# DakeQQ/Voice-Activity-Detection-VAD-ONNX

Hardware: NVIDIA B200
Metric: RTFx (audio-hours/sec) (higher is better)
Workload: dtype f32

## Files before the change

### voice-activity-detection-vad-onnx_b200/csrc/stft_tc.cu

```cuda
#include "tc_ptx.cuh"

namespace vadx {

constexpr int kStNPad = 80;
constexpr int kStTerms = 2;
constexpr int kStLead = 8;
constexpr int kStJ = 2;
constexpr int kStSlices = 2 * kStJ;
constexpr int kStStages = 3;
constexpr int kStLoaderWarps = 16;
constexpr int kStOutLd = 44;

struct StftTcArgs {
  const int16_t* X;
  int64_t in_stride;
  int64_t L;
  int64_t S;
  int n_frames, hop;
  int h16;
  int n_q;
  int tq;
  int rows;
  int slice_units;
  int n_st;
  const uint8_t* Wimg;
  float* P;
  int64_t ldp;
  int n_bins, kc, n_k16, n_tiles, vec_p;
  int pad_left;
  const float* mean;
  const int* mean_int;
  const float* dc;
  int n_edge_lo, t_edge_hi;
  float power_scale;
  int stage_out;
  unsigned backoff_ld, backoff_epi;
  int debug;
};

__device__ __forceinline__ uint32_t bf16x2_lo(uint32_t w) {
  const float a = __uint_as_float(0x4B000000u | (w & 0xffu)) - 8388608.0f;
  const float b = __uint_as_float(0x4B000000u | ((w >> 16) & 0xffu)) - 8388608.0f;
  return __byte_perm(__float_as_uint(a), __float_as_uint(b), 0x7632);
}
__device__ __forceinline__ uint32_t bf16x2_hi(uint32_t w) {
  const uint32_t ha = (((w >> 8) & 0xffu) ^ 0x80u);
  const uint32_t hb = (((w >> 24) & 0xffu) ^ 0x80u);
  const float a = fmaf(__uint_as_float(0x4B000000u | ha), 256.0f, -(8388608.0f + 128.0f) * 256.0f);
  const float b = fmaf(__uint_as_float(0x4B000000u | hb), 256.0f, -(8388608.0f + 128.0f) * 256.0f);
  return __byte_perm(__float_as_uint(a), __float_as_uint(b), 0x7632);
}

__device__ __forceinline__ uint32_t f16x2_lo(uint32_t w) {
  const uint32_t m = (w & 0x00ff00ffu) | 0x64006400u;
  uint32_t r;
  asm("sub.rn.f16x2 %0, %1, %2;" : "=r"(r) : "r"(m), "r"(0x64006400u));
  return r;
}
__device__ __forceinline__ uint32_t f16x2_hi(uint32_t w) {
  const uint32_t m = (((w >> 8) & 0x00ff00ffu) ^ 0x00800080u) | 0x64006400u;
  uint32_t r;
  asm("sub.rn.f16x2 %0, %1, %2;" : "=r"(r) : "r"(m), "r"(0x64806480u));
  asm("mul.rn.f16x2 %0, %1, %2;" : "=r"(r) : "r"(r), "r"(0x5c005c00u));
  return r;
}

__device__ __forceinline__ void split17(int d, float& hi, float& lo) {
  lo = __uint_as_float(0x4B000000u | (uint32_t)(d & 255)) - 8388608.0f;
  const uint32_t h = (uint32_t)((d >> 8) + 256);
  hi = fmaf(__uint_as_float(0x4B000000u | h), 256.0f, -(8388608.0f + 256.0f) * 256.0f);
}

template <bool EX, bool F16>
__global__ void __launch_bounds__((kStLoaderWarps + 5) * 32, 1) stft_power_tc_kernel(const StftTcArgs g) {
  constexpr int kStEpiWarp0 = kStLoaderWarps, kStMmaWarp = kStLoaderWarps + 4;
  extern __shared__ __align__(1024) uint8_t smem_raw[];
  uint8_t* w_smem = smem_raw;
  const uint32_t img_bytes = kStNPad * 128u;
  const int w_bytes = g.kc * kStTerms * (int)img_bytes;
  uint8_t* a_smem = w_smem + w_bytes;
  const uint32_t slice_bytes = (uint32_t)g.slice_units * 16u;
  const uint32_t term_bytes = kStSlices * slice_bytes;
  const uint32_t stage_bytes = 2u * term_bytes;
  uint64_t* bars = reinterpret_cast<uint64_t*>(a_smem + (size_t)kStStages * stage_bytes);
  uint32_t* tmem_slot = reinterpret_cast<uint32_t*>(bars + 13);
  float* out_stage = reinterpret_cast<float*>(bars + 16);

  const int warp = threadIdx.x >> 5, lane = threadIdx.x & 31;
  const uint32_t bar0 = smem_u32(bars);
  auto full_bar = [&](int s) { return bar0 + 8u * s; };
  auto empty_bar = [&](int s) { return bar0 + 8u * (4 + s); };
  auto tfull_bar = [&](int b) { return bar0 + 8u * (8 + b); };
  auto tempty_bar = [&](int b) { return bar0 + 8u * (10 + b); };
  const uint32_t wbar = bar0 + 8u * 12;
  constexpr int kAccN = 2 * kStNPad;
  constexpr uint32_t kTmemCols = 512;

  if (threadIdx.x == 0) {
    for (int s = 0; s < kStStages; ++s) {
      mbar_init(full_bar(s), kStLoaderWarps);
      mbar_init(empty_bar(s), 1);
    }
    for (int b = 0; b < 2; ++b) {
      mbar_init(tfull_bar(b), 1);
      mbar_init(tempty_bar(b), 4);
    }
    mbar_init(wbar, 1);
    asm volatile("fence.mbarrier_init.release.cluster;" ::: "memory");
  }
  if (warp == kStMmaWarp) {
    asm volatile("tcgen05.alloc.cta_group::1.sync.aligned.shared::cta.b32 [%0], %1;" ::"r"(smem_u32(tmem_slot)),
                 "r"(kTmemCols)
                 : "memory");
    asm volatile("tcgen05.relinquish_alloc_permit.cta_group::1.sync.aligned;" ::: "memory");
  }
  tc_fence_before();
  __syncthreads();
  tc_fence_after();
  const uint32_t tmem_base = *tmem_slot;
  const int ntile = blockIdx.y;

  if (warp == kStMmaWarp) {
    if (lane == 0) {
      mbar_expect_tx(wbar, (uint32_t)w_bytes);
      const uint8_t* src = g.Wimg + (size_t)ntile * w_bytes;
      for (int t = 0; t < g.kc * kStTerms; ++t) bulk_g2s(smem_u32(w_smem) + t * img_bytes, src + (size_t)t * img_bytes, img_bytes, wbar);
      mbar_wait(wbar, 0);
      const uint32_t idesc = F16 ? umma_idesc_f16(kAccN) : umma_idesc_bf16(kAccN);
      const uint64_t dw = umma_desc_sw128(smem_u32(w_smem));
      const uint64_t da0 = umma_desc_noswz(smem_u32(a_smem), slice_bytes, 128u);
      const uint32_t chunk_units = (kStTerms * img_bytes) >> 4, lo_units = term_bytes >> 4, stage_units = stage_bytes >> 4;
      const uint32_t col_units = (2u * slice_bytes) >> 4;
      const int h16 = g.h16, n_k16 = g.n_k16;
      const uint32_t lo_on = (g.debug & 4) ? 0u : 1u;
      constexpr bool kBurst = F16 && !EX;
      auto b_desc = [&](int k) { return dw + (uint64_t)((uint32_t)(k >> 2) * chunk_units + 2u * (uint32_t)(k & 3)); };
      int stage = 0;
      uint32_t phase = 0;
      int it = 0;
      for (int tile = blockIdx.x; tile < g.n_tiles; tile += gridDim.x, ++it) {
        const int b = it & 1;
        const uint32_t use = (uint32_t)(it >> 1);
        mbar_wait(tempty_bar(b), (use & 1u) ^ 1u);
        tc_fence_after();
        const uint32_t d_tmem = tmem_base + (uint32_t)(b * kAccN);
        for (int st = 0; st < g.n_st; ++st) {
          mbar_wait(full_bar(stage), phase);
          tc_fence_after();
          const uint64_t da_st = da0 + (uint64_t)stage * stage_units;
#pragma unroll
          for (int jj = 0; jj < kStJ; ++jj) {
            const int j = st * kStJ + jj;
            if (j >= h16) break;
            const uint64_t da_j = da_st + (uint64_t)jj * col_units;
            if (kBurst) {
              for (int q0 = 0, k = j; k < n_k16; q0 += 3, k += 3 * h16) {
                const int n_pairs = 1 + (k + h16 < n_k16 ? 1 : 0) + (k + 2 * h16 < n_k16 ? 1 : 0);
                umma_split_x3(d_tmem, da_j + (uint64_t)q0, 1u, lo_units, b_desc(k), b_desc(k + h16), b_desc(k + 2 * h16),
                              idesc, k ? 1u : 0u, n_pairs, lo_on);
              }
            } else {
              for (int q = 0, k = j; k < n_k16; ++q, k += h16) {
                const uint64_t da = da_j + (uint64_t)q;
                if (g.debug & 4) umma_bf16(d_tmem, da, b_desc(k), idesc, k ? 1u : 0u);
                else umma_x2(d_tmem, da, da + lo_units, b_desc(k), idesc, k ? 1u : 0u);
              }
            }
          }
          umma_commit(empty_bar(stage));
          if (++stage == kStStages) { stage = 0; phase ^= 1u; }
        }
        umma_commit(tfull_bar(b));
      }
    }
  } else if (warp < kStLoaderWarps) {
    constexpr int kRowsPerPass = kStLoaderWarps * 32 / kStSlices;
    constexpr int kPasses = 2;
    const int t = threadIdx.x;
    const int sl = t % kStSlices;
    const int r_in = t / kStSlices;
    const int16_t* xs_n[kPasses];
    int h0_n[kPasses];
    uint32_t rok_n = 0u;
    int tile_cached = -1;
    struct Seq { int tile, st; };
    auto valid = [&](const Seq& q) { return q.tile < g.n_tiles; };
    auto advance = [&](Seq& q) { if (++q.st == g.n_st) { q.st = 0; q.tile += gridDim.x; } };
    const int n_groups = 2 * g.h16;
    auto issue = [&](const Seq& q, uint4* raw, uint32_t& msk) {
      msk = 0u;
      if (q.tile != tile_cached) {
        rok_n = 0u;
#pragma unroll
        for (int pass = 0; pass < kPasses; ++pass) {
          const int r = pass * kRowsPerPass + r_in;
          const int64_t slot = (int64_t)q.tile * kTcBM + r;
          const int64_t s = slot / g.tq;
          const int h = (int)(slot - s * g.tq);
          const bool ok = r < g.rows && s < g.S;
          xs_n[pass] = g.X + (ok ? s : 0) * g.in_stride;
          h0_n[pass] = h * g.hop - (EX ? g.pad_left : 0) - kStLead;
          if (ok) rok_n |= 1u << pass;
        }
        tile_cached = q.tile;
      }
      const int grp = q.st * kStSlices + sl;
#pragma unroll
      for (int pass = 0; pass < kPasses; ++pass) {
        const int i0 = h0_n[pass] + 8 * grp;
        uint4 v = make_uint4(0u, 0u, 0u, 0u);
        if (((rok_n >> pass) & 1u) && grp < n_groups && i0 >= 0 && i0 + 7 < g.L) {
          v = __ldg(reinterpret_cast<const uint4*>(xs_n[pass] + i0));
          msk |= 1u << pass;
        }
        raw[pass] = v;
      }
    };
    int stage = 0;
    uint32_t phase = 0;
    int mi_c[kPasses];
#pragma unroll
    for (int pass = 0; pass < kPasses; ++pass) mi_c[pass] = 0;
    int tile_cached_c = -1;
    auto consume = [&](const Seq& q, const uint4* raw, uint32_t msk) {
      if (EX && g.mean_int && q.tile != tile_cached_c) {
#pragma unroll
        for (int pass = 0; pass < kPasses; ++pass) {
          const int64_t s = ((int64_t)q.tile * kTcBM + pass * kRowsPerPass + r_in) / g.tq;
          mi_c[pass] = s < g.S ? __ldg(g.mean_int + s) : 0;
        }
        tile_cached_c = q.tile;
      }
      mbar_wait(empty_bar(stage), phase ^ 1u, g.backoff_ld);
      uint8_t* st_hi = a_smem + (size_t)stage * stage_bytes + sl * slice_bytes;
      uint8_t* st_lo = st_hi + term_bytes;
      if (!(g.debug & 8) && q.st * kStSlices + sl < n_groups)
#pragma unroll
      for (int pass = 0; pass < kPasses; ++pass) {
        const int r = pass * kRowsPerPass + r_in;
        if (r >= g.rows) break;
        const uint32_t wds[4] = {raw[pass].x, raw[pass].y, raw[pass].z, raw[pass].w};
        uint32_t hi[4], lo[4];
        if (EX && g.mean_int) {
          const int mi = ((msk >> pass) & 1u) ? mi_c[pass] : 0;
#pragma unroll
          for (int j = 0; j < 4; ++j) {
            const uint32_t w = wds[j];
            const int a = ((int)(w << 16) >> 16) - mi;
            const int b = ((int)w >> 16) - mi;
            float ah, al, bh, bl;
            split17(a, ah, al);
            split17(b, bh, bl);
            hi[j] = __byte_perm(__float_as_uint(ah), __float_as_uint(bh), 0x7632);
            lo[j] = __byte_perm(__float_as_uint(al), __float_as_uint(bl), 0x7632);
          }
        } else {
#pragma unroll
        for (int j = 0; j < 4; ++j) {
          const uint32_t w = wds[j];
          hi[j] = F16 ? f16x2_hi(w) : bf16x2_hi(w);
          lo[j] = F16 ? f16x2_lo(w) : bf16x2_lo(w);
        }
        }
        *reinterpret_cast<uint4*>(st_hi + r * 16) = make_uint4(hi[0], hi[1], hi[2], hi[3]);
        *reinterpret_cast<uint4*>(st_lo + r * 16) = make_uint4(lo[0], lo[1], lo[2], lo[3]);
      }
      if (!(g.debug & 16)) fence_proxy_async();
      __syncwarp();
      if (lane == 0) mbar_arrive(full_bar(stage));
      if (++stage == kStStages) { stage = 0; phase ^= 1u; }
    };
    constexpr int kStBufs = EX ? 4 : 6;
    uint4 bufs[kStBufs][kPasses];
    uint32_t msks[kStBufs];
#pragma unroll
    for (int i = 0; i < kStBufs; ++i) msks[i] = 0u;
    Seq nxt{(int)blockIdx.x, 0}, cur{(int)blockIdx.x, 0};
#pragma unroll
    for (int i = 0; i < kStBufs - 1; ++i)
      if (valid(nxt)) { issue(nxt, bufs[i], msks[i]); advance(nxt); }
    while (valid(cur)) {
#pragma unroll
      for (int i = 0; i < kStBufs; ++i) {
        constexpr int kPrev = kStBufs - 1;
        if (valid(nxt)) { issue(nxt, bufs[(i + kPrev) % kStBufs], msks[(i + kPrev) % kStBufs]); advance(nxt); }
        consume(cur, bufs[i], msks[i]); advance(cur);
        if (!valid(cur)) break;
      }
    }
  } else {
    const int q = warp - kStEpiWarp0;
    int it = 0;
    const int f0 = ntile * (kStNPad / 2);
    for (int tile = blockIdx.x; tile < g.n_tiles; tile += gridDim.x, ++it) {
      const int b = it & 1;
      const uint32_t use = (uint32_t)(it >> 1);
      mbar_wait(tfull_bar(b), use & 1u, g.backoff_epi);
      tc_fence_after();
      const int64_t slot = (int64_t)tile * kTcBM + q * 32 + lane;
      const int64_t sidx = slot / g.tq;
      const int t = (int)(slot - sidx * g.tq);
      const bool row_ok = sidx < g.S && t < g.n_frames;
      const int64_t row = row_ok ? sidx * g.n_frames + t : -1;
      const uint32_t taddr = tmem_base + ((uint32_t)(q * 32) << 16) + (uint32_t)(b * kAccN);
      float* const my_out = out_stage + (size_t)q * 32 * kStOutLd;
      float m_row = 0.f, x_last = 0.f;
      const float* dc_row = nullptr;
      const float* tail_row = nullptr;
      if (EX && g.dc && row_ok) {
        const int n_edge = g.n_edge_lo + (g.n_frames - g.t_edge_hi);
        if (g.mean) {
          m_row = __ldg(g.mean + sidx);
          const int e = t < g.n_edge_lo ? 1 + t : (t >= g.t_edge_hi ? 1 + g.n_edge_lo + (t - g.t_edge_hi) : 0);
          dc_row = g.dc + ((size_t)e * gridDim.y + ntile) * kStNPad;
        }
        if (t >= g.t_edge_hi) {
          x_last = (float)((int)__ldg(g.X + sidx * g.in_stride + (g.L - 1)) - (g.mean_int ? __ldg(g.mean_int + sidx) : 0));
          tail_row = g.dc + ((size_t)(1 + n_edge + (t - g.t_edge_hi)) * gridDim.y + ntile) * kStNPad;
        }
      }
#pragma unroll
      for (int c0 = 0; c0 < kStNPad; c0 += 16) {
        float v[16], v2[16];
        tmem_ld16(taddr + (uint32_t)c0, v);
        tmem_ld16(taddr + (uint32_t)(kStNPad + c0), v2);
#pragma unroll
        for (int j = 0; j < 16; ++j) v[j] += v2[j];
        if (!row_ok || (g.debug & 1)) continue;
        if (EX && dc_row) {
#pragma unroll
          for (int j = 0; j < 16; ++j) v[j] = fmaf(-m_row, __ldg(dc_row + c0 + j), v[j]);
        }
        if (EX && tail_row) {
#pragma unroll
          for (int j = 0; j < 16; ++j) v[j] = fmaf(x_last, __ldg(tail_row + c0 + j), v[j]);
        }
        float* out = g.P + row * g.ldp + f0 + c0 / 2;
        float pw[8];
#pragma unroll
        for (int j = 0; j < 8; ++j) pw[j] = (v[2 * j] * v[2 * j] + v[2 * j + 1] * v[2 * j + 1]) * g.power_scale;
        const int fb = f0 + c0 / 2;
        if (g.stage_out) {
          float4* d4 = reinterpret_cast<float4*>(my_out + lane * kStOutLd + c0 / 2);
          d4[0] = make_float4(pw[0], pw[1], pw[2], pw[3]);
          d4[1] = make_float4(pw[4], pw[5], pw[6], pw[7]);
        } else if (g.vec_p && fb + 7 < g.n_bins) {
          reinterpret_cast<float4*>(out)[0] = make_float4(pw[0], pw[1], pw[2], pw[3]);
          reinterpret_cast<float4*>(out)[1] = make_float4(pw[4], pw[5], pw[6], pw[7]);
        } else {
#pragma unroll
          for (int j = 0; j < 8; ++j)
            if (fb + j < g.n_bins) out[j] = pw[j];
        }
      }
      tc_fence_before();
      __syncwarp();
      if (lane == 0) mbar_arrive(tempty_bar(b));
      if (g.stage_out && !(g.debug & 1)) {
        constexpr int kC4 = kStNPad / 8;
#pragma unroll
        for (int itr = 0; itr < kC4; ++itr) {
          const int idx = itr * 32 + lane;
          const int r = idx / kC4, c4 = idx - r * kC4;
          const long long grow = __shfl_sync(0xffffffffu, (long long)row, r);
          const int fbin = f0 + c4 * 4;
          if (grow >= 0 && fbin < g.n_bins) {
            const float4 val = *reinterpret_cast<const float4*>(my_out + r * kStOutLd + c4 * 4);
            float* out = g.P + grow * g.ldp + fbin;
            if (fbin + 3 < g.n_bins) {
              *reinterpret_cast<float4*>(out) = val;
            } else {
              out[0] = val.x;
              if (fbin + 1 < g.n_bins) out[1] = val.y;
              if (fbin + 2 < g.n_bins) out[2] = val.z;
            }
          }
        }
        __syncwarp();
      }
    }
  }
  tc_fence_before();
  __syncthreads();
  if (warp == kStMmaWarp) {
    tc_fence_after();
    asm volatile("tcgen05.dealloc.cta_group::1.sync.aligned.b32 %0, %1;" ::"r"(tmem_base), "r"(kTmemCols) : "memory");
  }
}

struct StftTcRing {
  int n_q, rows, slice_units;
  size_t bytes;
};
static StftTcRing stft_tc_ring(int n_k16, int h16) {
  StftTcRing r{};
  r.n_q = (n_k16 - 1) / h16 + 1;
  r.rows = kTcBM + r.n_q - 1;
  r.slice_units = r.rows + ((2 - r.rows % 4) + 4) % 4;
  r.bytes = (size_t)kStStages * 2 * kStSlices * r.slice_units * 16;
  return r;
}

struct StftTcShape {
  int kc, n_k16, n_ntiles;
  size_t tile_bytes, img_bytes, smem_bytes, stage_bytes;
  bool ok;
};
StftTcShape stft_tc_shape(int n_taps, int n_bins, int hop = 16) {
  StftTcShape s{};
  const int k_used = n_taps + kStLead;
  s.kc = (int)ceil_div(k_used, kTcBK);
  s.n_k16 = (int)ceil_div(k_used, 16);
  s.n_ntiles = (int)ceil_div(2 * n_bins, kStNPad);
  s.tile_bytes = (size_t)s.kc * kStTerms * kStNPad * 128;
  s.img_bytes = s.tile_bytes * s.n_ntiles;
  s.smem_bytes = s.tile_bytes + stft_tc_ring(s.n_k16, std::max(1, hop / 16)).bytes + 16 * 8;
  s.stage_bytes = (size_t)4 * 32 * kStOutLd * sizeof(float);
  s.ok = s.smem_bytes <= (size_t)kTcSmemBudget;
  return s;
}

}

using namespace vadx;

extern "C" int vadx_stft_tc_supported(int n_taps, int n_bins) { return stft_tc_shape(n_taps, n_bins).ok ? 1 : 0; }

extern "C" int vadx_pack_stft_basis_tc(const float* h_basis, int ld_basis, int n_taps, int n_bins, double preemph,
                                       double scale, void* h_img, size_t img_capacity, size_t* img_bytes) {
  return vadx_pack_stft_basis_tc_fmt(h_basis, ld_basis, n_taps, n_bins, preemph, scale, VADX_TC_FMT_BF16, h_img, img_capacity,
                                     img_bytes);
}

extern "C" int vadx_pack_stft_basis_tc_fmt(const float* h_basis, int ld_basis, int n_taps, int n_bins, double preemph,
                                           double scale, int operand_format, void* h_img, size_t img_capacity,
                                           size_t* img_bytes) {
  VADX_REQUIRE(h_basis && img_bytes && n_taps > 0 && n_bins > 0 && ld_basis >= 2 * n_bins,
               "vadx_pack_stft_basis_tc: bad argument");
  VADX_REQUIRE(operand_format == VADX_TC_FMT_BF16 || operand_format == VADX_TC_FMT_F16, "vadx_pack_stft_basis_tc: operand format %d",
               operand_format);
  const bool f16 = operand_format == VADX_TC_FMT_F16;
  StftTcShape s = stft_tc_shape(n_taps, n_bins);
  VADX_REQUIRE(s.ok, "vadx_pack_stft_basis_tc: %d taps x %d bins does not fit the tensor-core DFT", n_taps, n_bins);
  *img_bytes = s.img_bytes;
  if (!h_img) return VADX_OK;
  VADX_REQUIRE(img_capacity >= s.img_bytes, "vadx_pack_stft_basis_tc: image buffer too small");
  uint8_t* img = static_cast<uint8_t*>(h_img);
  memset(img, 0, s.img_bytes);
  const int n_cols = 2 * n_bins;
  const size_t term = (size_t)kStNPad * 128;
  for (int col = 0; col < n_cols; ++col) {
    const int nt = col / kStNPad, r = col % kStNPad;
    for (int k = 0; k < n_taps + kStLead; ++k) {
      const int n0 = k - kStLead, n1 = k - kStLead + 1;
      double v = 0.0;
      if (n0 >= 0 && n0 < n_taps) v += (double)h_basis[(size_t)n0 * ld_basis + col];
      if (n1 >= 0 && n1 < n_taps) v -= preemph * (double)h_basis[(size_t)n1 * ld_basis + col];
      v *= scale;
      const float f = (float)v;
      const uint16_t b0 = f16 ? f16_rn_host(f) : bf16_rn_host(f);
      const float r1 = (float)(v - (double)(f16 ? f16_to_f_host(b0) : bf16_to_f_host(b0)));
      const uint16_t b1 = f16 ? f16_rn_host(r1) : bf16_rn_host(r1);
      const int c = k / kTcBK, kk = k % kTcBK;
      uint8_t* base = img + (size_t)nt * s.tile_bytes + (size_t)(c * kStTerms) * term + sw128_offset(r, kk);
      memcpy(base, &b0, 2);
      memcpy(base + term, &b1, 2);
    }
  }
  return VADX_OK;
}

extern "C" int vadx_pack_stft_dc_tc(const float* h_basis, int ld_basis, int n_taps, int n_bins, double preemph, double scale,
                                    int64_t n_samples, int hop, int pad_left, int n_frames, float* h_tables,
                                    size_t capacity_floats, size_t* n_floats, int* n_edge_lo, int* t_edge_hi) {
  VADX_REQUIRE(h_basis && n_floats && n_edge_lo && t_edge_hi && n_taps > 0 && n_bins > 0 && hop > 0 && pad_left >= 0 &&
                   n_frames > 0 && ld_basis >= 2 * n_bins,
               "vadx_pack_stft_dc_tc: bad argument");
  StftTcShape s = stft_tc_shape(n_taps, n_bins);
  VADX_REQUIRE(s.ok, "vadx_pack_stft_dc_tc: shape not supported");
  int lo = 0;
  while (lo < n_frames && (int64_t)lo * hop - pad_left < 1) ++lo;
  int hi = n_frames;
  while (hi > lo && (int64_t)(hi - 1) * hop - pad_left + n_taps - 1 >= n_samples) --hi;
  *n_edge_lo = lo;
  *t_edge_hi = hi;
  const int n_edge = lo + (n_frames - hi);
  const size_t ncp = (size_t)s.n_ntiles * kStNPad;
  *n_floats = (size_t)(1 + n_edge + (n_frames - hi)) * ncp;
  if (!h_tables) return VADX_OK;
  VADX_REQUIRE(capacity_floats >= *n_floats, "vadx_pack_stft_dc_tc: table buffer too small");
  memset(h_tables, 0, *n_floats * sizeof(float));
  auto fill = [&](float* row, int64_t origin, bool interior) {
    for (int col = 0; col < 2 * n_bins; ++col) {
      double acc = 0.0;
      for (int n = 0; n < n_taps; ++n) {
        const int64_t i = origin + n;
        double coef = interior ? 1.0 - preemph : (i < 0 || i >= n_samples ? 0.0 : (i == 0 ? 1.0 : 1.0 - preemph));
        acc += coef * (double)h_basis[(size_t)n * ld_basis + col];
      }
      row[col] = (float)(acc * scale);
    }
  };
  fill(h_tables, 0, true);
  int e = 1;
  for (int t = 0; t < lo; ++t, ++e) fill(h_tables + (size_t)e * ncp, (int64_t)t * hop - pad_left, false);
  for (int t = hi; t < n_frames; ++t, ++e) fill(h_tables + (size_t)e * ncp, (int64_t)t * hop - pad_left, false);
  for (int t = hi; t < n_frames; ++t, ++e) {
    const int64_t n_l = n_samples - ((int64_t)t * hop - pad_left);
    if (n_l < 0 || n_l >= n_taps) continue;
    float* row = h_tables + (size_t)e * ncp;
    for (int col = 0; col < 2 * n_bins; ++col) row[col] = (float)(preemph * scale * (double)h_basis[(size_t)n_l * ld_basis + col]);
  }
  return VADX_OK;
}

namespace vadx {
__global__ void __launch_bounds__(256) stream_mean_i16_kernel(const int16_t* __restrict__ x, int64_t in_stride, int64_t n,
                                                              float* __restrict__ mean_frac, int* __restrict__ mean_int) {
  const int64_t s = blockIdx.x;
  const int16_t* p = x + s * in_stride;
  long long acc = 0;
  for (int64_t i = threadIdx.x; i < n; i += blockDim.x) acc += (long long)__ldg(p + i);
  __shared__ long long part[8];
#pragma unroll
  for (int off = 16; off > 0; off >>= 1) acc += __shfl_xor_sync(0xffffffffu, acc, off);
  if ((threadIdx.x & 31) == 0) part[threadIdx.x >> 5] = acc;
  __syncthreads();
  if (threadIdx.x == 0) {
    long long t = 0;
    for (int w = 0; w < 8; ++w) t += part[w];
    const double m = (double)t / (double)n;
    const int mi = (int)llrint(m);
    mean_int[s] = mi;
    mean_frac[s] = (float)(m - (double)mi);
  }
}
}

extern "C" int vadx_stream_mean_i16(const int16_t* d_audio, int64_t in_stride, int64_t n_samples, int64_t n_streams,
                                    float* d_mean_frac, int32_t* d_mean_int, void* stream) {
  StageTimer _timer(VADX_STAGE_PREP, (cudaStream_t)stream, "stream_mean_i16_kernel", 2.0 * n_streams * n_samples);
  VADX_REQUIRE(d_audio && d_mean_frac && d_mean_int && n_samples > 0 && in_stride >= n_samples && n_streams >= 0,
               "vadx_stream_mean_i16: bad argument");
  if (n_streams == 0) return VADX_OK;
  stream_mean_i16_kernel<<<(unsigned)n_streams, 256, 0, (cudaStream_t)stream>>>(d_audio, in_stride, n_samples, d_mean_frac,
                                                                                d_mean_int);
  return after_launch("vadx_stream_mean_i16");
}

extern "C" int vadx_stft_power_tc_i16(const int16_t* d_audio, int64_t in_stride, int64_t n_samples, int64_t n_streams,
                                      int n_frames, int hop, int n_taps, const void* d_img, int n_bins, float* d_power,
                                      int64_t ld_power, void* stream) {
  VADX_REQUIRE((int64_t)(n_frames - 1) * hop + n_taps <= n_samples,
               "vadx_stft_power_tc_i16: frames must lie inside the %lld samples of a stream", (long long)n_samples);
  return vadx_stft_power_tc_i16_ex(d_audio, in_stride, n_samples, n_streams, n_frames, hop, n_taps, d_img, n_bins, d_power,
                                   ld_power, 0, nullptr, nullptr, nullptr, 0, n_frames, 1.0f, VADX_TC_FMT_BF16, stream);
}

extern "C" int vadx_stft_power_tc_i16_ex(const int16_t* d_audio, int64_t in_stride, int64_t n_samples, int64_t n_streams,
                                         int n_frames, int hop, int n_taps, const void* d_img, int n_bins, float* d_power,
                                         int64_t ld_power, int pad_left, const float* d_mean_frac, const int32_t* d_mean_int,
                                         const float* d_dc_tables, int n_edge_lo, int t_edge_hi, float power_scale,
                                         int operand_format, void* stream) {
  const float* d_mean = d_mean_frac;
  VADX_REQUIRE(operand_format == VADX_TC_FMT_BF16 || (operand_format == VADX_TC_FMT_F16 && !d_mean_frac),
               "vadx_stft_power_tc_i16: fp16 operands cannot carry the mean-removed (17-bit) samples");
  VADX_REQUIRE((d_mean_frac == nullptr) == (d_mean_int == nullptr), "vadx_stft_power_tc_i16: mean needs both its parts");
  StageTimer _timer(VADX_STAGE_STFT, (cudaStream_t)stream, "stft_power_tc_kernel",
                    2.0 * n_streams * n_samples + 4.0 * n_streams * n_frames * n_bins,
                    2.0 * n_streams * n_frames * n_taps * 2.0 * n_bins);
  VADX_REQUIRE(d_audio && d_img && d_power, "vadx_stft_power_tc_i16: null pointer");
  VADX_REQUIRE(n_streams >= 0 && n_frames > 0 && hop > 0 && n_taps > 0 && n_bins > 0 && ld_power >= n_bins,
               "vadx_stft_power_tc_i16: bad shape");
  VADX_REQUIRE(in_stride >= n_samples && pad_left >= 0 && (pad_left % 8) == 0 && (n_samples % 8) == 0,
               "vadx_stft_power_tc_i16: stride shorter than the stream, or pad_left / n_samples not a multiple of 8");
  const bool leaves_stream = pad_left > 0 || (int64_t)(n_frames - 1) * hop - pad_left + n_taps > n_samples;
  VADX_REQUIRE(!(d_mean || leaves_stream) || (d_dc_tables && n_edge_lo >= 0 && t_edge_hi >= n_edge_lo && t_edge_hi <= n_frames),
               "vadx_stft_power_tc_i16: padded frames / DC removal need the tables of vadx_pack_stft_dc_tc");
  VADX_REQUIRE((hop % 16) == 0,
               "vadx_stft_power_tc_i16: hop %d is not a multiple of 16 samples (frames are read as shifted rows of 16-sample "
               "hop slices); use vadx_stft_power_f32", hop);
  VADX_REQUIRE((in_stride % 8) == 0 && aligned16(d_audio) && aligned16(d_img),
               "vadx_stft_power_tc_i16: stream stride must be a multiple of 8 samples, pointers 16-byte aligned");
  StftTcShape s = stft_tc_shape(n_taps, n_bins, hop);
  VADX_REQUIRE(s.ok, "vadx_stft_power_tc_i16: shape not supported");
  if (n_streams == 0) return VADX_OK;
  static PerDevice per_device;
  int n_sm = 148;
  VADX_TRY(per_device.ensure(&n_sm, [] {
    cudaError_t e = cudaSuccess;
    auto opt_in = [&](auto kern) {
      if (e == cudaSuccess) e = cudaFuncSetAttribute(kern, cudaFuncAttributeMaxDynamicSharedMemorySize, kTcSmemBudget);
    };
    opt_in(stft_power_tc_kernel<false, false>);
    opt_in(stft_power_tc_kernel<true, false>);
    opt_in(stft_power_tc_kernel<false, true>);
    opt_in(stft_power_tc_kernel<true, true>);
    return e;
  }));
  const StftTcRing ring = stft_tc_ring(s.n_k16, hop / 16);
  StftTcArgs g{};
  g.X = d_audio; g.in_stride = in_stride; g.L = n_samples; g.S = n_streams; g.n_frames = n_frames; g.hop = hop;
  g.h16 = hop / 16; g.n_q = ring.n_q; g.tq = n_frames + ring.n_q - 1; g.rows = ring.rows; g.slice_units = ring.slice_units;
  g.n_st = (int)ceil_div(g.h16, kStJ);
  g.Wimg = static_cast<const uint8_t*>(d_img); g.P = d_power; g.ldp = ld_power;
  g.n_bins = n_bins; g.kc = s.kc; g.n_k16 = s.n_k16;
  g.pad_left = pad_left; g.mean = d_mean; g.mean_int = d_mean_int; g.dc = d_dc_tables; g.power_scale = power_scale; g.n_edge_lo = n_edge_lo; g.t_edge_hi = t_edge_hi;
  g.vec_p = ((ld_power & 3) == 0) && aligned16(d_power);
  {
    static const int dbg = ab_env("VADX_TC_DEBUG", 0);
    g.debug = dbg;
  }
  static const int opt = ab_env("VADX_ST_OPT", 2);
  {
    static const int bl = ab_env("VADX_TC_BACKOFF_LD", 64);
    static const int be = ab_env("VADX_TC_BACKOFF_EPI", 256);
    g.backoff_ld = (unsigned)bl; g.backoff_epi = (unsigned)be;
  }
  g.stage_out = ((opt & 2) && g.vec_p && s.smem_bytes + s.stage_bytes <= (size_t)kTcSmemBudget) ? 1 : 0;
  const size_t smem = s.smem_bytes + (g.stage_out ? s.stage_bytes : 0);
  int64_t tiles = ceil_div(n_streams * g.tq, kTcBM);
  VADX_REQUIRE(tiles <= 0x7fffffffLL, "vadx_stft_power_tc_i16: too many rows");
  g.n_tiles = (int)tiles;
  int per = std::max(1, n_sm / s.n_ntiles);
  dim3 grid((unsigned)std::min<int64_t>(tiles, per), (unsigned)s.n_ntiles);
  const bool ex = leaves_stream || d_mean, f16 = operand_format == VADX_TC_FMT_F16;
  constexpr int kThreads = (kStLoaderWarps + 5) * 32;
  if (ex && f16) stft_power_tc_kernel<true, true><<<grid, kThreads, smem, (cudaStream_t)stream>>>(g);
  else if (ex) stft_power_tc_kernel<true, false><<<grid, kThreads, smem, (cudaStream_t)stream>>>(g);
  else if (f16) stft_power_tc_kernel<false, true><<<grid, kThreads, smem, (cudaStream_t)stream>>>(g);
  else stft_power_tc_kernel<false, false><<<grid, kThreads, smem, (cudaStream_t)stream>>>(g);
  return after_launch("vadx_stft_power_tc_i16");
}
```

### voice-activity-detection-vad-onnx_b200/csrc/tc_ptx.cuh

```cuda
#pragma once
#include "common.cuh"

namespace vadx {

constexpr int kTcBM = 128;
constexpr int kTcBK = 64;
constexpr int kTcTileBytes = kTcBM * 128;
constexpr int kTcSmemBudget = 227 * 1024;

__device__ __forceinline__ uint32_t smem_u32(const void* p) { return (uint32_t)__cvta_generic_to_shared(p); }

__device__ __forceinline__ void mbar_init(uint32_t bar, uint32_t count) {
  asm volatile("mbarrier.init.shared::cta.b64 [%0], %1;" ::"r"(bar), "r"(count));
}
__device__ __forceinline__ void mbar_arrive(uint32_t bar) {
  asm volatile("mbarrier.arrive.shared::cta.b64 _, [%0];" ::"r"(bar) : "memory");
}
__device__ __forceinline__ void mbar_expect_tx(uint32_t bar, uint32_t bytes) {
  asm volatile("mbarrier.arrive.expect_tx.shared::cta.b64 _, [%0], %1;" ::"r"(bar), "r"(bytes) : "memory");
}
__device__ __forceinline__ bool mbar_try_wait(uint32_t bar, uint32_t parity) {
  uint32_t ok;
  asm volatile(
      "{\n.reg .pred p;\nmbarrier.try_wait.parity.shared::cta.b64 p, [%1], %2;\nselp.u32 %0, 1, 0, p;\n}\n"
      : "=r"(ok)
      : "r"(bar), "r"(parity)
      : "memory");
  return ok != 0;
}
__device__ __forceinline__ void mbar_wait(uint32_t bar, uint32_t parity, unsigned backoff_ns = 0) {
  if (mbar_try_wait(bar, parity)) return;
  const long long t0 = clock64();
  while (!mbar_try_wait(bar, parity)) {
    if (backoff_ns) __nanosleep(backoff_ns);
    if (clock64() - t0 > 20000000000LL) __trap();
  }
}
__device__ __forceinline__ void fence_proxy_async() { asm volatile("fence.proxy.async.shared::cta;" ::: "memory"); }
__device__ __forceinline__ void tc_fence_before() { asm volatile("tcgen05.fence::before_thread_sync;" ::: "memory"); }
__device__ __forceinline__ void tc_fence_after() { asm volatile("tcgen05.fence::after_thread_sync;" ::: "memory"); }

__device__ __forceinline__ void bulk_g2s(uint32_t dst, const void* src, uint32_t bytes, uint32_t bar) {
  asm volatile("cp.async.bulk.shared::cluster.global.mbarrier::complete_tx::bytes [%0], [%1], %2, [%3];" ::"r"(dst),
               "l"(src), "r"(bytes), "r"(bar)
               : "memory");
}

__device__ __forceinline__ void bulk_s2g(void* dst, uint32_t src, uint32_t bytes) {
  asm volatile("cp.async.bulk.global.shared::cta.bulk_group [%0], [%1], %2;" ::"l"(dst), "r"(src), "r"(bytes) : "memory");
}

__device__ __forceinline__ uint64_t umma_desc_sw128(uint32_t smem_addr) {
  uint64_t d = 0;
  d |= (uint64_t)((smem_addr & 0x3FFFFu) >> 4);
  d |= (uint64_t)1 << 16;
  d |= (uint64_t)(1024 >> 4) << 32;
  d |= (uint64_t)1 << 46;
  d |= (uint64_t)2 << 61;
  return d;
}
__device__ __forceinline__ uint64_t umma_desc_noswz(uint32_t smem_addr, uint32_t lbo, uint32_t sbo) {
  uint64_t d = 0;
  d |= (uint64_t)((smem_addr & 0x3FFFFu) >> 4);
  d |= (uint64_t)((lbo >> 4) & 0x3FFFu) << 16;
  d |= (uint64_t)((sbo >> 4) & 0x3FFFu) << 32;
  d |= (uint64_t)1 << 46;
  return d;
}
__device__ __forceinline__ uint32_t umma_idesc_bf16(int n) {
  return (1u << 4) | (1u << 7) | (1u << 10) | ((uint32_t)(n >> 3) << 17) | ((uint32_t)(kTcBM >> 4) << 24);
}
__device__ __forceinline__ uint32_t umma_idesc_f16(int n) {
  return (1u << 4) | ((uint32_t)(n >> 3) << 17) | ((uint32_t)(kTcBM >> 4) << 24);
}
__device__ __forceinline__ void umma_bf16(uint32_t tmem_d, uint64_t adesc, uint64_t bdesc, uint32_t idesc,
                                          uint32_t accumulate) {
  asm volatile(
      "{\n.reg .pred p;\nsetp.ne.b32 p, %4, 0;\ntcgen05.mma.cta_group::1.kind::f16 [%0], %1, %2, %3, p;\n}\n" ::"r"(tmem_d),
      "l"(adesc), "l"(bdesc), "r"(idesc), "r"(accumulate)
      : "memory");
}
__device__ __forceinline__ void umma_k64(uint32_t tmem_d, uint64_t adesc, uint64_t bdesc, uint32_t idesc,
                                         uint32_t accumulate_first, int n_steps) {
  asm volatile(
      "{\n"
      ".reg .pred p0, pt, q1, q2, q3;\n"
      ".reg .b64 a1, a2, a3, b1, b2, b3;\n"
      "setp.ne.b32 p0, %4, 0;\n"
      "setp.eq.b32 pt, 0, 0;\n"
      "setp.gt.s32 q1, %5, 1;\n"
      "setp.gt.s32 q2, %5, 2;\n"
      "setp.gt.s32 q3, %5, 3;\n"
      "add.u64 a1, %1, 2;\n"
      "add.u64 a2, %1, 4;\n"
      "add.u64 a3, %1, 6;\n"
      "add.u64 b1, %2, 2;\n"
      "add.u64 b2, %2, 4;\n"
      "add.u64 b3, %2, 6;\n"
      "tcgen05.mma.cta_group::1.kind::f16 [%0], %1, %2, %3, p0;\n"
      "@q1 tcgen05.mma.cta_group::1.kind::f16 [%0], a1, b1, %3, pt;\n"
      "@q2 tcgen05.mma.cta_group::1.kind::f16 [%0], a2, b2, %3, pt;\n"
      "@q3 tcgen05.mma.cta_group::1.kind::f16 [%0], a3, b3, %3, pt;\n"
      "}\n" ::"r"(tmem_d),
      "l"(adesc), "l"(bdesc), "r"(idesc), "r"(accumulate_first), "r"(n_steps)
      : "memory");
}
__device__ __forceinline__ void umma_x2(uint32_t tmem_d, uint64_t adesc0, uint64_t adesc1, uint64_t bdesc, uint32_t idesc,
                                        uint32_t accumulate_first) {
  asm volatile(
      "{\n.reg .pred p, pt;\n"
      "setp.ne.b32 p, %5, 0;\n"
      "setp.eq.b32 pt, 0, 0;\n"
      "tcgen05.mma.cta_group::1.kind::f16 [%0], %1, %3, %4, p;\n"
      "tcgen05.mma.cta_group::1.kind::f16 [%0], %2, %3, %4, pt;\n"
      "}\n" ::"r"(tmem_d),
      "l"(adesc0), "l"(adesc1), "l"(bdesc), "r"(idesc), "r"(accumulate_first)
      : "memory");
}
__device__ __forceinline__ void umma_split_x3(uint32_t tmem_d, uint64_t a, uint32_t a_step, uint32_t a_lo, uint64_t b0,
                                              uint64_t b1, uint64_t b2, uint32_t idesc, uint32_t accumulate_first,
                                              int n_pairs, uint32_t lo_on) {
  asm volatile(
      "{\n"
      ".reg .pred p0, pt, q1, q2, l0, l1, l2;\n"
      ".reg .b64 st, lo, a0h, a1, a1h, a2, a2h;\n"
      "setp.ne.b32 p0, %7, 0;\n"
      "setp.eq.b32 pt, 0, 0;\n"
      "setp.gt.s32 q1, %8, 1;\n"
      "setp.gt.s32 q2, %8, 2;\n"
      "setp.ne.b32 l0, %9, 0;\n"
      "and.pred l1, l0, q1;\n"
      "and.pred l2, l0, q2;\n"
      "cvt.u64.u32 st, %2;\n"
      "cvt.u64.u32 lo, %3;\n"
      "add.u64 a0h, %1, lo;\n"
      "add.u64 a1, %1, st;\n"
      "add.u64 a1h, a1, lo;\n"
      "add.u64 a2, a1, st;\n"
      "add.u64 a2h, a2, lo;\n"
      "tcgen05.mma.cta_group::1.kind::f16 [%0], %1, %4, %6, p0;\n"
      "@l0 tcgen05.mma.cta_group::1.kind::f16 [%0], a0h, %4, %6, pt;\n"
      "@q1 tcgen05.mma.cta_group::1.kind::f16 [%0], a1, %5, %6, pt;\n"
      "@l1 tcgen05.mma.cta_group::1.kind::f16 [%0], a1h, %5, %6, pt;\n"
      "@q2 tcgen05.mma.cta_group::1.kind::f16 [%0], a2, %10, %6, pt;\n"
      "@l2 tcgen05.mma.cta_group::1.kind::f16 [%0], a2h, %10, %6, pt;\n"
      "}\n" ::"r"(tmem_d),
      "l"(a), "r"(a_step), "r"(a_lo), "l"(b0), "l"(b1), "r"(idesc), "r"(accumulate_first), "r"(n_pairs), "r"(lo_on),
      "l"(b2)
      : "memory");
}
__device__ __forceinline__ void umma_commit(uint32_t bar) {
  asm volatile("tcgen05.commit.cta_group::1.mbarrier::arrive::one.shared::cluster.b64 [%0];" ::"r"(bar) : "memory");
}
__device__ __forceinline__ void tmem_ld16(uint32_t taddr, float* v) {
  uint32_t r[16];
  asm volatile(
      "tcgen05.ld.sync.aligned.32x32b.x16.b32 {%0,%1,%2,%3,%4,%5,%6,%7,%8,%9,%10,%11,%12,%13,%14,%15}, [%16];"
      : "=r"(r[0]), "=r"(r[1]), "=r"(r[2]), "=r"(r[3]), "=r"(r[4]), "=r"(r[5]), "=r"(r[6]), "=r"(r[7]), "=r"(r[8]),
        "=r"(r[9]), "=r"(r[10]), "=r"(r[11]), "=r"(r[12]), "=r"(r[13]), "=r"(r[14]), "=r"(r[15])
      : "r"(taddr));
  asm volatile("tcgen05.wait::ld.sync.aligned;" ::: "memory");
#pragma unroll
  for (int i = 0; i < 16; ++i) v[i] = __uint_as_float(r[i]);
}

__device__ __forceinline__ void tmem_ld8_issue(uint32_t taddr, uint32_t* r) {
  asm volatile("tcgen05.ld.sync.aligned.32x32b.x8.b32 {%0,%1,%2,%3,%4,%5,%6,%7}, [%8];"
               : "=r"(r[0]), "=r"(r[1]), "=r"(r[2]), "=r"(r[3]), "=r"(r[4]), "=r"(r[5]), "=r"(r[6]), "=r"(r[7])
               : "r"(taddr));
}
__device__ __forceinline__ void tmem_ld8_finish(uint32_t* r) {
  asm volatile("tcgen05.wait::ld.sync.aligned;"
               : "+r"(r[0]), "+r"(r[1]), "+r"(r[2]), "+r"(r[3]), "+r"(r[4]), "+r"(r[5]), "+r"(r[6]), "+r"(r[7])
               :
               : "memory");
}

__device__ __forceinline__ void tmem_ld8(uint32_t taddr, float* v) {
  uint32_t r[8];
  asm volatile("tcgen05.ld.sync.aligned.32x32b.x8.b32 {%0,%1,%2,%3,%4,%5,%6,%7}, [%8];"
               : "=r"(r[0]), "=r"(r[1]), "=r"(r[2]), "=r"(r[3]), "=r"(r[4]), "=r"(r[5]), "=r"(r[6]), "=r"(r[7])
               : "r"(taddr));
  asm volatile("tcgen05.wait::ld.sync.aligned;" ::: "memory");
#pragma unroll
  for (int i = 0; i < 8; ++i) v[i] = __uint_as_float(r[i]);
}

__device__ __forceinline__ void l2_prefetch(const void* p, uint32_t bytes) {
  asm volatile("cp.async.bulk.prefetch.L2.global [%0], %1;" ::"l"(p), "r"(bytes) : "memory");
}

__device__ __forceinline__ void ldg256_nc(const float* p, float4& a, float4& b) {
  asm volatile("ld.global.nc.v8.f32 {%0,%1,%2,%3,%4,%5,%6,%7}, [%8];"
               : "=f"(a.x), "=f"(a.y), "=f"(a.z), "=f"(a.w), "=f"(b.x), "=f"(b.y), "=f"(b.z), "=f"(b.w)
               : "l"(p));
}

__device__ __forceinline__ void tmem_ld32(uint32_t taddr, float* v) {
  uint32_t r[32];
  asm volatile(
      "tcgen05.ld.sync.aligned.32x32b.x32.b32 "
      "{%0,%1,%2,%3,%4,%5,%6,%7,%8,%9,%10,%11,%12,%13,%14,%15,%16,%17,%18,%19,%20,%21,%22,%23,%24,%25,%26,%27,%28,%29,%30,%31}, [%32];"
      : "=r"(r[0]), "=r"(r[1]), "=r"(r[2]), "=r"(r[3]), "=r"(r[4]), "=r"(r[5]), "=r"(r[6]), "=r"(r[7]), "=r"(r[8]),
        "=r"(r[9]), "=r"(r[10]), "=r"(r[11]), "=r"(r[12]), "=r"(r[13]), "=r"(r[14]), "=r"(r[15]), "=r"(r[16]),
        "=r"(r[17]), "=r"(r[18]), "=r"(r[19]), "=r"(r[20]), "=r"(r[21]), "=r"(r[22]), "=r"(r[23]), "=r"(r[24]),
        "=r"(r[25]), "=r"(r[26]), "=r"(r[27]), "=r"(r[28]), "=r"(r[29]), "=r"(r[30]), "=r"(r[31])
      : "r"(taddr));
  asm volatile("tcgen05.wait::ld.sync.aligned;" ::: "memory");
#pragma unroll
  for (int i = 0; i < 32; ++i) v[i] = __uint_as_float(r[i]);
}

__device__ __forceinline__ void split2(float a, float b, uint32_t& hi, uint32_t& lo) {
  asm("cvt.rn.bf16x2.f32 %0, %1, %2;" : "=r"(hi) : "f"(b), "f"(a));
  float ah = __uint_as_float(hi << 16), bh = __uint_as_float(hi & 0xffff0000u);
  float al = a - ah, bl = b - bh;
  asm("cvt.rn.bf16x2.f32 %0, %1, %2;" : "=r"(lo) : "f"(bl), "f"(al));
}


static inline uint16_t bf16_rn_host(float f) {
  uint32_t u;
  memcpy(&u, &f, 4);
  if ((u & 0x7f800000u) == 0x7f800000u) return (uint16_t)(u >> 16);
  u += 0x7fffu + ((u >> 16) & 1u);
  return (uint16_t)(u >> 16);
}
static inline float bf16_to_f_host(uint16_t h) {
  uint32_t u = (uint32_t)h << 16;
  float f;
  memcpy(&f, &u, 4);
  return f;
}
static inline uint16_t f16_rn_host(float f) {
  uint32_t u;
  memcpy(&u, &f, 4);
  const uint32_t sign = (u >> 16) & 0x8000u;
  const int32_t exp = (int32_t)((u >> 23) & 0xffu) - 127 + 15;
  uint32_t man = u & 0x7fffffu;
  if (((u >> 23) & 0xffu) == 0xffu) return (uint16_t)(sign | 0x7c00u | (man ? 0x200u : 0u));
  if (exp >= 31) return (uint16_t)(sign | 0x7c00u);
  if (exp <= 0) {
    if (exp < -10) return (uint16_t)sign;
    man |= 0x800000u;
    const int shift = 14 - exp;
    uint32_t h = man >> shift;
    const uint32_t rem = man & ((1u << shift) - 1u), halfway = 1u << (shift - 1);
    if (rem > halfway || (rem == halfway && (h & 1u))) ++h;
    return (uint16_t)(sign | h);
  }
  uint32_t h = ((uint32_t)exp << 10) | (man >> 13);
  const uint32_t rem = man & 0x1fffu;
  if (rem > 0x1000u || (rem == 0x1000u && (h & 1u))) ++h;
  return (uint16_t)(sign | h);
}
static inline float f16_to_f_host(uint16_t h) {
  const uint32_t sign = (uint32_t)(h & 0x8000u) << 16;
  const uint32_t exp = (h >> 10) & 0x1fu, man = h & 0x3ffu;
  float f;
  if (exp == 0) {
    f = ldexpf((float)man, -24);
    uint32_t u;
    memcpy(&u, &f, 4);
    u |= sign;
    memcpy(&f, &u, 4);
    return f;
  }
  const uint32_t u = exp == 31 ? (sign | 0x7f800000u | (man << 13)) : (sign | ((exp - 15 + 127) << 23) | (man << 13));
  memcpy(&f, &u, 4);
  return f;
}
static inline size_t sw128_offset(int r, int kk) {
  return (size_t)(r / 8) * 1024 + (size_t)(r % 8) * 128 + (size_t)(((kk / 8) ^ (r % 8)) * 16) + (size_t)(kk % 8) * 2;
}

}
```

Baseline: 373.1.

## Move STFT tensor-core kernel to 2-CTA cluster UMMA with split weight halves

Converts the STFT power kernel to cta_group::2 tcgen05 MMA across a 2-CTA cluster. Each CTA loads half the weight image and its own row tile, and the leader issues M=256 MMAs with multicast commits. The change also makes the pipeline stage count runtime-sized to the smem budget (up to 6), replaces the padded 80-column layout with a variable bin count, and moves the burst choice to a runtime flag. The aim is to halve per-CTA weight smem and the issue overhead per row. The cost is cross-CTA barrier traffic and cluster scheduling constraints.

```diff
diff --git a/voice-activity-detection-vad-onnx_b200/csrc/stft_tc.cu b/voice-activity-detection-vad-onnx_b200/csrc/stft_tc.cu
--- a/voice-activity-detection-vad-onnx_b200/csrc/stft_tc.cu
+++ b/voice-activity-detection-vad-onnx_b200/csrc/stft_tc.cu
@@ -1,15 +1,18 @@
+#include <mutex>
+
 #include "tc_ptx.cuh"
 
 namespace vadx {
 
-constexpr int kStNPad = 80;
+constexpr int kStMaxBins = 64;
 constexpr int kStTerms = 2;
 constexpr int kStLead = 8;
 constexpr int kStJ = 2;
 constexpr int kStSlices = 2 * kStJ;
-constexpr int kStStages = 3;
+constexpr int kStMinStages = 3, kStMaxStages = 6;
+constexpr int kStBarWords = 2 * kStMaxStages + 6;
 constexpr int kStLoaderWarps = 16;
-constexpr int kStOutLd = 44;
+constexpr uint32_t kStAccCols = 256;
 
 struct StftTcArgs {
   const int16_t* X;
@@ -23,10 +26,13 @@
   int rows;
   int slice_units;
   int n_st;
+  int n_stages;
   const uint8_t* Wimg;
   float* P;
   int64_t ldp;
-  int n_bins, kc, n_k16, n_tiles, vec_p;
+  int n_bins, kc, n_k16, vec_p;
+  int bins;
+  int n_ptiles;
   int pad_left;
   const float* mean;
   const int* mean_int;
@@ -34,6 +40,8 @@
   int n_edge_lo, t_edge_hi;
   float power_scale;
   int stage_out;
+  int out_ld;
+  int burst;
   unsigned backoff_ld, backoff_epi;
   int debug;
 };
@@ -71,106 +79,115 @@
   hi = fmaf(__uint_as_float(0x4B000000u | h), 256.0f, -(8388608.0f + 256.0f) * 256.0f);
 }
 
+
 template <bool EX, bool F16>
-__global__ void __launch_bounds__((kStLoaderWarps + 5) * 32, 1) stft_power_tc_kernel(const StftTcArgs g) {
+__global__ void __cluster_dims__(2, 1, 1) __launch_bounds__((kStLoaderWarps + 5) * 32, 1)
+    stft_power_tc_kernel(const StftTcArgs g) {
   constexpr int kStEpiWarp0 = kStLoaderWarps, kStMmaWarp = kStLoaderWarps + 4;
   extern __shared__ __align__(1024) uint8_t smem_raw[];
   uint8_t* w_smem = smem_raw;
-  const uint32_t img_bytes = kStNPad * 128u;
-  const int w_bytes = g.kc * kStTerms * (int)img_bytes;
+  const int ncol = 2 * g.bins;
+  const uint32_t img_bytes = (uint32_t)ncol * 128u;
+  const int w_bytes = g.kc * (int)img_bytes;
   uint8_t* a_smem = w_smem + w_bytes;
   const uint32_t slice_bytes = (uint32_t)g.slice_units * 16u;
   const uint32_t term_bytes = kStSlices * slice_bytes;
   const uint32_t stage_bytes = 2u * term_bytes;
-  uint64_t* bars = reinterpret_cast<uint64_t*>(a_smem + (size_t)kStStages * stage_bytes);
-  uint32_t* tmem_slot = reinterpret_cast<uint32_t*>(bars + 13);
-  float* out_stage = reinterpret_cast<float*>(bars + 16);
+  uint64_t* bars = reinterpret_cast<uint64_t*>(a_smem + (size_t)g.n_stages * stage_bytes);
+  uint32_t* tmem_slot = reinterpret_cast<uint32_t*>(bars + kStBarWords - 1);
+  float* out_stage = reinterpret_cast<float*>(bars + kStBarWords);
 
   const int warp = threadIdx.x >> 5, lane = threadIdx.x & 31;
+  const uint32_t rank = cluster_ctarank();
+  const int pair = blockIdx.x >> 1, n_pairs = gridDim.x >> 1;
   const uint32_t bar0 = smem_u32(bars);
+  const uint32_t lead_bar0 = mapa_shared(bar0, 0);
   auto full_bar = [&](int s) { return bar0 + 8u * s; };
-  auto empty_bar = [&](int s) { return bar0 + 8u * (4 + s); };
-  auto tfull_bar = [&](int b) { return bar0 + 8u * (8 + b); };
-  auto tempty_bar = [&](int b) { return bar0 + 8u * (10 + b); };
-  const uint32_t wbar = bar0 + 8u * 12;
-  constexpr int kAccN = 2 * kStNPad;
-  constexpr uint32_t kTmemCols = 512;
+  auto empty_bar = [&](int s) { return bar0 + 8u * (kStMaxStages + s); };
+  auto tfull_bar = [&](int b) { return bar0 + 8u * (2 * kStMaxStages + b); };
+  auto tempty_bar = [&](int b) { return bar0 + 8u * (2 * kStMaxStages + 2 + b); };
+  const uint32_t wbar = bar0 + 8u * (2 * kStMaxStages + 4);
 
   if (threadIdx.x == 0) {
-    for (int s = 0; s < kStStages; ++s) {
-      mbar_init(full_bar(s), kStLoaderWarps);
+    for (int s = 0; s < g.n_stages; ++s) {
+      mbar_init(full_bar(s), 2 * kStLoaderWarps);
       mbar_init(empty_bar(s), 1);
     }
     for (int b = 0; b < 2; ++b) {
       mbar_init(tfull_bar(b), 1);
-      mbar_init(tempty_bar(b), 4);
+      mbar_init(tempty_bar(b), 8);
     }
-    mbar_init(wbar, 1);
+    mbar_init(wbar, rank == 0 ? 2 : 1);
     asm volatile("fence.mbarrier_init.release.cluster;" ::: "memory");
   }
   if (warp == kStMmaWarp) {
-    asm volatile("tcgen05.alloc.cta_group::1.sync.aligned.shared::cta.b32 [%0], %1;" ::"r"(smem_u32(tmem_slot)),
-                 "r"(kTmemCols)
+    asm volatile("tcgen05.alloc.cta_group::2.sync.aligned.shared::cta.b32 [%0], %1;" ::"r"(smem_u32(tmem_slot)),
+                 "r"(2 * kStAccCols)
                  : "memory");
-    asm volatile("tcgen05.relinquish_alloc_permit.cta_group::1.sync.aligned;" ::: "memory");
+    asm volatile("tcgen05.relinquish_alloc_permit.cta_group::2.sync.aligned;" ::: "memory");
   }
   tc_fence_before();
-  __syncthreads();
+  cluster_sync();
   tc_fence_after();
-  const uint32_t tmem_base = *tmem_slot;
   const int ntile = blockIdx.y;
 
   if (warp == kStMmaWarp) {
     if (lane == 0) {
       mbar_expect_tx(wbar, (uint32_t)w_bytes);
-      const uint8_t* src = g.Wimg + (size_t)ntile * w_bytes;
-      for (int t = 0; t < g.kc * kStTerms; ++t) bulk_g2s(smem_u32(w_smem) + t * img_bytes, src + (size_t)t * img_bytes, img_bytes, wbar);
-      mbar_wait(wbar, 0);
-      const uint32_t idesc = F16 ? umma_idesc_f16(kAccN) : umma_idesc_bf16(kAccN);
-      const uint64_t dw = umma_desc_sw128(smem_u32(w_smem));
-      const uint64_t da0 = umma_desc_noswz(smem_u32(a_smem), slice_bytes, 128u);
-      const uint32_t chunk_units = (kStTerms * img_bytes) >> 4, lo_units = term_bytes >> 4, stage_units = stage_bytes >> 4;
-      const uint32_t col_units = (2u * slice_bytes) >> 4;
-      const int h16 = g.h16, n_k16 = g.n_k16;
-      const uint32_t lo_on = (g.debug & 4) ? 0u : 1u;
-      constexpr bool kBurst = F16 && !EX;
-      auto b_desc = [&](int k) { return dw + (uint64_t)((uint32_t)(k >> 2) * chunk_units + 2u * (uint32_t)(k & 3)); };
-      int stage = 0;
-      uint32_t phase = 0;
-      int it = 0;
-      for (int tile = blockIdx.x; tile < g.n_tiles; tile += gridDim.x, ++it) {
-        const int b = it & 1;
-        const uint32_t use = (uint32_t)(it >> 1);
-        mbar_wait(tempty_bar(b), (use & 1u) ^ 1u);
-        tc_fence_after();
-        const uint32_t d_tmem = tmem_base + (uint32_t)(b * kAccN);
-        for (int st = 0; st < g.n_st; ++st) {
-          mbar_wait(full_bar(stage), phase);
+      bulk_g2s(smem_u32(w_smem), g.Wimg + ((size_t)ntile * kStTerms + rank) * w_bytes, (uint32_t)w_bytes, wbar);
+      if (rank != 0) {
+        mbar_wait(wbar, 0);
+        mbar_arrive_cluster(lead_bar0 + (wbar - bar0));
+      } else {
+        mbar_wait(wbar, 0);
+        const uint32_t tmem_base = *tmem_slot;
+        const int n4 = 4 * g.bins;
+        const uint32_t idesc = F16 ? umma_idesc_f16(n4, 2 * kTcBM) : umma_idesc_bf16(n4, 2 * kTcBM);
+        const uint64_t dw = umma_desc_sw128(smem_u32(w_smem));
+        const uint64_t da0 = umma_desc_noswz(smem_u32(a_smem), slice_bytes, 128u);
+        const uint32_t chunk_units = img_bytes >> 4, lo_units = term_bytes >> 4, stage_units = stage_bytes >> 4;
+        const uint32_t col_units = (2u * slice_bytes) >> 4;
+        const int h16 = g.h16, n_k16 = g.n_k16;
+        const uint32_t lo_on = (g.debug & 4) ? 0u : 1u;
+        const bool burst = g.burst != 0;
+        auto b_desc = [&](int k) { return dw + (uint64_t)((uint32_t)(k >> 2) * chunk_units + 2u * (uint32_t)(k & 3)); };
+        int stage = 0;
+        uint32_t phase = 0;
+        int it = 0;
+        for (int pt = pair; pt < g.n_ptiles; pt += n_pairs, ++it) {
+          const int b = it & 1;
+          const uint32_t use = (uint32_t)(it >> 1);
+          mbar_wait(tempty_bar(b), (use & 1u) ^ 1u);
           tc_fence_after();
-          const uint64_t da_st = da0 + (uint64_t)stage * stage_units;
-#pragma unroll
-          for (int jj = 0; jj < kStJ; ++jj) {
-            const int j = st * kStJ + jj;
-            if (j >= h16) break;
-            const uint64_t da_j = da_st + (uint64_t)jj * col_units;
-            if (kBurst) {
-              for (int q0 = 0, k = j; k < n_k16; q0 += 3, k += 3 * h16) {
-                const int n_pairs = 1 + (k + h16 < n_k16 ? 1 : 0) + (k + 2 * h16 < n_k16 ? 1 : 0);
-                umma_split_x3(d_tmem, da_j + (uint64_t)q0, 1u, lo_units, b_desc(k), b_desc(k + h16), b_desc(k + 2 * h16),
-                              idesc, k ? 1u : 0u, n_pairs, lo_on);
-              }
-            } else {
-              for (int q = 0, k = j; k < n_k16; ++q, k += h16) {
-                const uint64_t da = da_j + (uint64_t)q;
-                if (g.debug & 4) umma_bf16(d_tmem, da, b_desc(k), idesc, k ? 1u : 0u);
-                else umma_x2(d_tmem, da, da + lo_units, b_desc(k), idesc, k ? 1u : 0u);
+          const uint32_t d_tmem = tmem_base + (uint32_t)b * kStAccCols;
+          for (int st = 0; st < g.n_st; ++st) {
+            mbar_wait(full_bar(stage), phase);
+            tc_fence_after();
+            const uint64_t da_st = da0 + (uint64_t)stage * stage_units;
+#pragma unroll
+            for (int jj = 0; jj < kStJ; ++jj) {
+              const int j = st * kStJ + jj;
+              if (j >= h16) break;
+              const uint64_t da_j = da_st + (uint64_t)jj * col_units;
+              if (burst) {
+                for (int q0 = 0, k = j; k < n_k16; q0 += 3, k += 3 * h16) {
+                  const int n_pairs_k = 1 + (k + h16 < n_k16 ? 1 : 0) + (k + 2 * h16 < n_k16 ? 1 : 0);
+                  umma_pair_split_x3(d_tmem, da_j + (uint64_t)q0, 1u, lo_units, b_desc(k), b_desc(k + h16),
+                                     b_desc(k + 2 * h16), idesc, k ? 1u : 0u, n_pairs_k, lo_on);
+                }
+              } else {
+                for (int q = 0, k = j; k < n_k16; ++q, k += h16) {
+                  const uint64_t da = da_j + (uint64_t)q;
+                  if (g.debug & 4) umma_pair(d_tmem, da, b_desc(k), idesc, k ? 1u : 0u);
+                  else umma_pair_x2(d_tmem, da, da + lo_units, b_desc(k), idesc, k ? 1u : 0u);
+                }
               }
             }
+            umma_pair_commit_mc(empty_bar(stage));
+            if (++stage == g.n_stages) { stage = 0; phase ^= 1u; }
           }
-          umma_commit(empty_bar(stage));
-          if (++stage == kStStages) { stage = 0; phase ^= 1u; }
-        }
-        umma_commit(tfull_bar(b));
+          umma_pair_commit_mc(tfull_bar(b));
+        }
       }
     }
   } else if (warp < kStLoaderWarps) {
@@ -184,8 +201,8 @@
     uint32_t rok_n = 0u;
     int tile_cached = -1;
     struct Seq { int tile, st; };
-    auto valid = [&](const Seq& q) { return q.tile < g.n_tiles; };
-    auto advance = [&](Seq& q) { if (++q.st == g.n_st) { q.st = 0; q.tile += gridDim.x; } };
+    auto valid = [&](const Seq& q) { return q.tile < g.n_ptiles; };
+    auto advance = [&](Seq& q) { if (++q.st == g.n_st) { q.st = 0; q.tile += n_pairs; } };
     const int n_groups = 2 * g.h16;
     auto issue = [&](const Seq& q, uint4* raw, uint32_t& msk) {
       msk = 0u;
@@ -194,7 +211,7 @@
 #pragma unroll
         for (int pass = 0; pass < kPasses; ++pass) {
           const int r = pass * kRowsPerPass + r_in;
-          const int64_t slot = (int64_t)q.tile * kTcBM + r;
+          const int64_t slot = (2 * (int64_t)q.tile + rank) * kTcBM + r;
           const int64_t s = slot / g.tq;
           const int h = (int)(slot - s * g.tq);
           const bool ok = r < g.rows && s < g.S;
@@ -226,7 +243,7 @@
       if (EX && g.mean_int && q.tile != tile_cached_c) {
 #pragma unroll
         for (int pass = 0; pass < kPasses; ++pass) {
-          const int64_t s = ((int64_t)q.tile * kTcBM + pass * kRowsPerPass + r_in) / g.tq;
+          const int64_t s = ((2 * (int64_t)q.tile + rank) * kTcBM + pass * kRowsPerPass + r_in) / g.tq;
           mi_c[pass] = s < g.S ? __ldg(g.mean_int + s) : 0;
         }
         tile_cached_c = q.tile;
@@ -267,15 +284,15 @@
       }
       if (!(g.debug & 16)) fence_proxy_async();
       __syncwarp();
-      if (lane == 0) mbar_arrive(full_bar(stage));
-      if (++stage == kStStages) { stage = 0; phase ^= 1u; }
+      if (lane == 0) mbar_arrive_cluster(lead_bar0 + (full_bar(stage) - bar0));
+      if (++stage == g.n_stages) { stage = 0; phase ^= 1u; }
     };
     constexpr int kStBufs = EX ? 4 : 6;
     uint4 bufs[kStBufs][kPasses];
     uint32_t msks[kStBufs];
 #pragma unroll
     for (int i = 0; i < kStBufs; ++i) msks[i] = 0u;
-    Seq nxt{(int)blockIdx.x, 0}, cur{(int)blockIdx.x, 0};
+    Seq nxt{pair, 0}, cur{pair, 0};
 #pragma unroll
     for (int i = 0; i < kStBufs - 1; ++i)
       if (valid(nxt)) { issue(nxt, bufs[i], msks[i]); advance(nxt); }
@@ -290,20 +307,21 @@
     }
   } else {
     const int q = warp - kStEpiWarp0;
+    const uint32_t tmem_base = *tmem_slot;
     int it = 0;
-    const int f0 = ntile * (kStNPad / 2);
-    for (int tile = blockIdx.x; tile < g.n_tiles; tile += gridDim.x, ++it) {
+    const int f0 = ntile * g.bins;
+    for (int pt = pair; pt < g.n_ptiles; pt += n_pairs, ++it) {
       const int b = it & 1;
       const uint32_t use = (uint32_t)(it >> 1);
       mbar_wait(tfull_bar(b), use & 1u, g.backoff_epi);
       tc_fence_after();
-      const int64_t slot = (int64_t)tile * kTcBM + q * 32 + lane;
+      const int64_t slot = (2 * (int64_t)pt + rank) * kTcBM + q * 32 + lane;
       const int64_t sidx = slot / g.tq;
       const int t = (int)(slot - sidx * g.tq);
       const bool row_ok = sidx < g.S && t < g.n_frames;
       const int64_t row = row_ok ? sidx * g.n_frames + t : -1;
-      const uint32_t taddr = tmem_base + ((uint32_t)(q * 32) << 16) + (uint32_t)(b * kAccN);
-      float* const my_out = out_stage + (size_t)q * 32 * kStOutLd;
+      const uint32_t taddr = tmem_base + ((uint32_t)(q * 32) << 16) + (uint32_t)b * kStAccCols;
+      float* const my_out = out_stage + (size_t)q * 32 * g.out_ld;
       float m_row = 0.f, x_last = 0.f;
       const float* dc_row = nullptr;
       const float* tail_row = nullptr;
@@ -312,60 +330,68 @@
         if (g.mean) {
           m_row = __ldg(g.mean + sidx);
           const int e = t < g.n_edge_lo ? 1 + t : (t >= g.t_edge_hi ? 1 + g.n_edge_lo + (t - g.t_edge_hi) : 0);
-          dc_row = g.dc + ((size_t)e * gridDim.y + ntile) * kStNPad;
+          dc_row = g.dc + ((size_t)e * gridDim.y + ntile) * ncol;
         }
         if (t >= g.t_edge_hi) {
           x_last = (float)((int)__ldg(g.X + sidx * g.in_stride + (g.L - 1)) - (g.mean_int ? __ldg(g.mean_int + sidx) : 0));
-          tail_row = g.dc + ((size_t)(1 + n_edge + (t - g.t_edge_hi)) * gridDim.y + ntile) * kStNPad;
-        }
-      }
-#pragma unroll
-      for (int c0 = 0; c0 < kStNPad; c0 += 16) {
-        float v[16], v2[16];
-        tmem_ld16(taddr + (uint32_t)c0, v);
-        tmem_ld16(taddr + (uint32_t)(kStNPad + c0), v2);
-#pragma unroll
-        for (int j = 0; j < 16; ++j) v[j] += v2[j];
-        if (!row_ok || (g.debug & 1)) continue;
+          tail_row = g.dc + ((size_t)(1 + n_edge + (t - g.t_edge_hi)) * gridDim.y + ntile) * ncol;
+        }
+      }
+      auto emit = [&](int c0, const uint32_t* r0, const uint32_t* r1) {
+        float v[8];
+#pragma unroll
+        for (int j = 0; j < 8; ++j) v[j] = __uint_as_float(r0[j]) + __uint_as_float(r1[j]);
+        if (!row_ok || (g.debug & 1)) return;
         if (EX && dc_row) {
 #pragma unroll
-          for (int j = 0; j < 16; ++j) v[j] = fmaf(-m_row, __ldg(dc_row + c0 + j), v[j]);
+          for (int j = 0; j < 8; ++j) v[j] = fmaf(-m_row, __ldg(dc_row + c0 + j), v[j]);
         }
         if (EX && tail_row) {
 #pragma unroll
-          for (int j = 0; j < 16; ++j) v[j] = fmaf(x_last, __ldg(tail_row + c0 + j), v[j]);
-        }
-        float* out = g.P + row * g.ldp + f0 + c0 / 2;
-        float pw[8];
-#pragma unroll
-        for (int j = 0; j < 8; ++j) pw[j] = (v[2 * j] * v[2 * j] + v[2 * j + 1] * v[2 * j + 1]) * g.power_scale;
+          for (int j = 0; j < 8; ++j) v[j] = fmaf(x_last, __ldg(tail_row + c0 + j), v[j]);
+        }
+        float pw[4];
+#pragma unroll
+        for (int j = 0; j < 4; ++j) pw[j] = (v[2 * j] * v[2 * j] + v[2 * j + 1] * v[2 * j + 1]) * g.power_scale;
         const int fb = f0 + c0 / 2;
+        float* out = g.P + row * g.ldp + fb;
         if (g.stage_out) {
-          float4* d4 = reinterpret_cast<float4*>(my_out + lane * kStOutLd + c0 / 2);
-          d4[0] = make_float4(pw[0], pw[1], pw[2], pw[3]);
-          d4[1] = make_float4(pw[4], pw[5], pw[6], pw[7]);
-        } else if (g.vec_p && fb + 7 < g.n_bins) {
-          reinterpret_cast<float4*>(out)[0] = make_float4(pw[0], pw[1], pw[2], pw[3]);
-          reinterpret_cast<float4*>(out)[1] = make_float4(pw[4], pw[5], pw[6], pw[7]);
+          *reinterpret_cast<float4*>(my_out + lane * g.out_ld + c0 / 2) = make_float4(pw[0], pw[1], pw[2], pw[3]);
+        } else if (g.vec_p && fb + 3 < g.n_bins) {
+          *reinterpret_cast<float4*>(out) = make_float4(pw[0], pw[1], pw[2], pw[3]);
         } else {
 #pragma unroll
-          for (int j = 0; j < 8; ++j)
+          for (int j = 0; j < 4; ++j)
             if (fb + j < g.n_bins) out[j] = pw[j];
         }
+      };
+      for (int c0 = 0; c0 < ncol; c0 += 16) {
+        uint32_t r0[16], r1[16];
+        const bool two = c0 + 8 < ncol;
+        tmem_ld8_issue(taddr + (uint32_t)c0, r0);
+        tmem_ld8_issue(taddr + (uint32_t)(ncol + c0), r1);
+        if (two) {
+          tmem_ld8_issue(taddr + (uint32_t)(c0 + 8), r0 + 8);
+          tmem_ld8_issue(taddr + (uint32_t)(ncol + c0 + 8), r1 + 8);
+          tmem_ld8_finish(r0 + 8);
+          tmem_ld8_finish(r1 + 8);
+        }
+        tmem_ld8_finish(r0);
+        tmem_ld8_finish(r1);
+        emit(c0, r0, r1);
+        if (two) emit(c0 + 8, r0 + 8, r1 + 8);
       }
       tc_fence_before();
       __syncwarp();
-      if (lane == 0) mbar_arrive(tempty_bar(b));
+      if (lane == 0) mbar_arrive_cluster(lead_bar0 + (tempty_bar(b) - bar0));
       if (g.stage_out && !(g.debug & 1)) {
-        constexpr int kC4 = kStNPad / 8;
-#pragma unroll
-        for (int itr = 0; itr < kC4; ++itr) {
-          const int idx = itr * 32 + lane;
-          const int r = idx / kC4, c4 = idx - r * kC4;
+        const int c4n = g.bins / 4;
+        for (int idx = lane; idx < 32 * c4n; idx += 32) {
+          const int r = idx / c4n, c4 = idx - r * c4n;
           const long long grow = __shfl_sync(0xffffffffu, (long long)row, r);
           const int fbin = f0 + c4 * 4;
           if (grow >= 0 && fbin < g.n_bins) {
-            const float4 val = *reinterpret_cast<const float4*>(my_out + r * kStOutLd + c4 * 4);
+            const float4 val = *reinterpret_cast<const float4*>(my_out + r * g.out_ld + c4 * 4);
             float* out = g.P + grow * g.ldp + fbin;
             if (fbin + 3 < g.n_bins) {
               *reinterpret_cast<float4*>(out) = val;
@@ -381,29 +407,29 @@
     }
   }
   tc_fence_before();
-  __syncthreads();
+  cluster_sync();
   if (warp == kStMmaWarp) {
     tc_fence_after();
-    asm volatile("tcgen05.dealloc.cta_group::1.sync.aligned.b32 %0, %1;" ::"r"(tmem_base), "r"(kTmemCols) : "memory");
+    asm volatile("tcgen05.dealloc.cta_group::2.sync.aligned.b32 %0, %1;" ::"r"(*tmem_slot), "r"(2 * kStAccCols) : "memory");
   }
 }
 
 struct StftTcRing {
   int n_q, rows, slice_units;
-  size_t bytes;
+  size_t stage_bytes;
 };
 static StftTcRing stft_tc_ring(int n_k16, int h16) {
   StftTcRing r{};
   r.n_q = (n_k16 - 1) / h16 + 1;
   r.rows = kTcBM + r.n_q - 1;
   r.slice_units = r.rows + ((2 - r.rows % 4) + 4) % 4;
-  r.bytes = (size_t)kStStages * 2 * kStSlices * r.slice_units * 16;
+  r.stage_bytes = (size_t)2 * kStSlices * r.slice_units * 16;
   return r;
 }
 
 struct StftTcShape {
-  int kc, n_k16, n_ntiles;
-  size_t tile_bytes, img_bytes, smem_bytes, stage_bytes;
+  int kc, n_k16, n_ntiles, bins, out_ld;
+  size_t term_bytes, img_bytes, smem_bytes, stage_bytes;
   bool ok;
 };
 StftTcShape stft_tc_shape(int n_taps, int n_bins, int hop = 16) {
@@ -411,11 +437,13 @@
   const int k_used = n_taps + kStLead;
   s.kc = (int)ceil_div(k_used, kTcBK);
   s.n_k16 = (int)ceil_div(k_used, 16);
-  s.n_ntiles = (int)ceil_div(2 * n_bins, kStNPad);
-  s.tile_bytes = (size_t)s.kc * kStTerms * kStNPad * 128;
-  s.img_bytes = s.tile_bytes * s.n_ntiles;
-  s.smem_bytes = s.tile_bytes + stft_tc_ring(s.n_k16, std::max(1, hop / 16)).bytes + 16 * 8;
-  s.stage_bytes = (size_t)4 * 32 * kStOutLd * sizeof(float);
+  s.n_ntiles = (int)ceil_div(n_bins, kStMaxBins);
+  s.bins = (int)ceil_div(ceil_div(n_bins, s.n_ntiles), 4) * 4;
+  s.out_ld = s.bins | 4;
+  s.term_bytes = (size_t)s.kc * 2 * s.bins * 128;
+  s.img_bytes = s.term_bytes * kStTerms * s.n_ntiles;
+  s.smem_bytes = s.term_bytes + kStMinStages * stft_tc_ring(s.n_k16, std::max(1, hop / 16)).stage_bytes + kStBarWords * 8;
+  s.stage_bytes = (size_t)4 * 32 * s.out_ld * sizeof(float);
   s.ok = s.smem_bytes <= (size_t)kTcSmemBudget;
   return s;
 }
@@ -447,10 +475,10 @@
   VADX_REQUIRE(img_capacity >= s.img_bytes, "vadx_pack_stft_basis_tc: image buffer too small");
   uint8_t* img = static_cast<uint8_t*>(h_img);
   memset(img, 0, s.img_bytes);
-  const int n_cols = 2 * n_bins;
-  const size_t term = (size_t)kStNPad * 128;
+  const int n_cols = 2 * n_bins, ncol = 2 * s.bins;
+  const size_t chunk = (size_t)ncol * 128;
   for (int col = 0; col < n_cols; ++col) {
-    const int nt = col / kStNPad, r = col % kStNPad;
+    const int nt = col / ncol, r = col % ncol;
     for (int k = 0; k < n_taps + kStLead; ++k) {
       const int n0 = k - kStLead, n1 = k - kStLead + 1;
       double v = 0.0;
@@ -462,9 +490,9 @@
       const float r1 = (float)(v - (double)(f16 ? f16_to_f_host(b0) : bf16_to_f_host(b0)));
       const uint16_t b1 = f16 ? f16_rn_host(r1) : bf16_rn_host(r1);
       const int c = k / kTcBK, kk = k % kTcBK;
-      uint8_t* base = img + (size_t)nt * s.tile_bytes + (size_t)(c * kStTerms) * term + sw128_offset(r, kk);
+      uint8_t* base = img + (size_t)nt * kStTerms * s.term_bytes + (size_t)c * chunk + sw128_offset(r, kk);
       memcpy(base, &b0, 2);
-      memcpy(base + term, &b1, 2);
+      memcpy(base + s.term_bytes, &b1, 2);
     }
   }
   return VADX_OK;
@@ -485,7 +513,7 @@
   *n_edge_lo = lo;
   *t_edge_hi = hi;
   const int n_edge = lo + (n_frames - hi);
-  const size_t ncp = (size_t)s.n_ntiles * kStNPad;
+  const size_t ncp = (size_t)s.n_ntiles * 2 * s.bins;
   *n_floats = (size_t)(1 + n_edge + (n_frames - hi)) * ncp;
   if (!h_tables) return VADX_OK;
   VADX_REQUIRE(capacity_floats >= *n_floats, "vadx_pack_stft_dc_tc: table buffer too small");
@@ -546,6 +574,44 @@
   stream_mean_i16_kernel<<<(unsigned)n_streams, 256, 0, (cudaStream_t)stream>>>(d_audio, in_stride, n_samples, d_mean_frac,
                                                                                 d_mean_int);
   return after_launch("vadx_stream_mean_i16");
+}
+
+constexpr int kStThreads = (kStLoaderWarps + 5) * 32;
+
+template <bool EX, bool F16>
+static int stft_tc_pairs(size_t smem, int* pairs) {
+  static std::mutex mu;
+  static size_t smem_of[PerDevice::kMaxDevices] = {};
+  static int pairs_of[PerDevice::kMaxDevices] = {};
+  int dev = 0;
+  cudaError_t e = cudaGetDevice(&dev);
+  if (e != cudaSuccess) return cuda_fail(e, "cudaGetDevice");
+  VADX_REQUIRE(dev >= 0 && dev < PerDevice::kMaxDevices, "device ordinal %d out of range", dev);
+  std::lock_guard<std::mutex> lk(mu);
+  if (smem_of[dev] != smem) {
+    cudaLaunchConfig_t cfg{};
+    cfg.gridDim = dim3(2, 1, 1);
+    cfg.blockDim = dim3(kStThreads, 1, 1);
+    cfg.dynamicSmemBytes = smem;
+    int n = 0;
+    e = cudaOccupancyMaxActiveClusters(&n, stft_power_tc_kernel<EX, F16>, &cfg);
+    if (e != cudaSuccess) return cuda_fail(e, "cudaOccupancyMaxActiveClusters");
+    VADX_REQUIRE(n > 0, "vadx_stft_power_tc_i16: no CTA pair with %zu bytes of shared memory fits the device", smem);
+    smem_of[dev] = smem;
+    pairs_of[dev] = n;
+  }
+  *pairs = pairs_of[dev];
+  return VADX_OK;
+}
+
+template <bool EX, bool F16>
+static int stft_tc_launch(const StftTcArgs& g, int n_ntiles, size_t smem, cudaStream_t st) {
+  int pairs = 0;
+  VADX_TRY((stft_tc_pairs<EX, F16>(smem, &pairs)));
+  const int per = std::min(g.n_ptiles, std::max(1, pairs / n_ntiles));
+  const dim3 grid((unsigned)(2 * per), (unsigned)n_ntiles);
+  stft_power_tc_kernel<EX, F16><<<grid, kStThreads, smem, st>>>(g);
+  return after_launch("vadx_stft_power_tc_i16");
 }
 
 extern "C" int vadx_stft_power_tc_i16(const int16_t* d_audio, int64_t in_stride, int64_t n_samples, int64_t n_streams,
@@ -586,8 +652,7 @@
   VADX_REQUIRE(s.ok, "vadx_stft_power_tc_i16: shape not supported");
   if (n_streams == 0) return VADX_OK;
   static PerDevice per_device;
-  int n_sm = 148;
-  VADX_TRY(per_device.ensure(&n_sm, [] {
+  VADX_TRY(per_device.ensure(nullptr, [] {
     cudaError_t e = cudaSuccess;
     auto opt_in = [&](auto kern) {
       if (e == cudaSuccess) e = cudaFuncSetAttribute(kern, cudaFuncAttributeMaxDynamicSharedMemorySize, kTcSmemBudget);
@@ -604,7 +669,7 @@
   g.h16 = hop / 16; g.n_q = ring.n_q; g.tq = n_frames + ring.n_q - 1; g.rows = ring.rows; g.slice_units = ring.slice_units;
   g.n_st = (int)ceil_div(g.h16, kStJ);
   g.Wimg = static_cast<const uint8_t*>(d_img); g.P = d_power; g.ldp = ld_power;
-  g.n_bins = n_bins; g.kc = s.kc; g.n_k16 = s.n_k16;
+  g.n_bins = n_bins; g.kc = s.kc; g.n_k16 = s.n_k16; g.bins = s.bins; g.out_ld = s.out_ld;
   g.pad_left = pad_left; g.mean = d_mean; g.mean_int = d_mean_int; g.dc = d_dc_tables; g.power_scale = power_scale; g.n_edge_lo = n_edge_lo; g.t_edge_hi = t_edge_hi;
   g.vec_p = ((ld_power & 3) == 0) && aligned16(d_power);
   {
@@ -618,17 +683,19 @@
     g.backoff_ld = (unsigned)bl; g.backoff_epi = (unsigned)be;
   }
   g.stage_out = ((opt & 2) && g.vec_p && s.smem_bytes + s.stage_bytes <= (size_t)kTcSmemBudget) ? 1 : 0;
-  const size_t smem = s.smem_bytes + (g.stage_out ? s.stage_bytes : 0);
-  int64_t tiles = ceil_div(n_streams * g.tq, kTcBM);
+  const size_t fixed = s.term_bytes + kStBarWords * 8 + (g.stage_out ? s.stage_bytes : 0);
+  static const int max_stages = std::min(kStMaxStages, std::max(kStMinStages, ab_env("VADX_ST_STAGES", kStMaxStages)));
+  g.n_stages = (int)std::min<size_t>(max_stages, ((size_t)kTcSmemBudget - fixed) / ring.stage_bytes);
+  const size_t smem = fixed + (size_t)g.n_stages * ring.stage_bytes;
+  const int64_t tiles = ceil_div(n_streams * g.tq, kTcBM);
   VADX_REQUIRE(tiles <= 0x7fffffffLL, "vadx_stft_power_tc_i16: too many rows");
-  g.n_tiles = (int)tiles;
-  int per = std::max(1, n_sm / s.n_ntiles);
-  dim3 grid((unsigned)std::min<int64_t>(tiles, per), (unsigned)s.n_ntiles);
+  g.n_ptiles = (int)ceil_div(tiles, 2);
   const bool ex = leaves_stream || d_mean, f16 = operand_format == VADX_TC_FMT_F16;
-  constexpr int kThreads = (kStLoaderWarps + 5) * 32;
-  if (ex && f16) stft_power_tc_kernel<true, true><<<grid, kThreads, smem, (cudaStream_t)stream>>>(g);
-  else if (ex) stft_power_tc_kernel<true, false><<<grid, kThreads, smem, (cudaStream_t)stream>>>(g);
-  else if (f16) stft_power_tc_kernel<false, true><<<grid, kThreads, smem, (cudaStream_t)stream>>>(g);
-  else stft_power_tc_kernel<false, false><<<grid, kThreads, smem, (cudaStream_t)stream>>>(g);
-  return after_launch("vadx_stft_power_tc_i16");
-}
+  static const int burst = ab_env("VADX_ST_BURST", -1);
+  g.burst = burst >= 0 ? burst : (f16 && !ex ? 1 : 0);
+  cudaStream_t st = (cudaStream_t)stream;
+  if (ex && f16) return stft_tc_launch<true, true>(g, s.n_ntiles, smem, st);
+  if (ex) return stft_tc_launch<true, false>(g, s.n_ntiles, smem, st);
+  if (f16) return stft_tc_launch<false, true>(g, s.n_ntiles, smem, st);
+  return stft_tc_launch<false, false>(g, s.n_ntiles, smem, st);
+}
diff --git a/voice-activity-detection-vad-onnx_b200/csrc/tc_ptx.cuh b/voice-activity-detection-vad-onnx_b200/csrc/tc_ptx.cuh
--- a/voice-activity-detection-vad-onnx_b200/csrc/tc_ptx.cuh
+++ b/voice-activity-detection-vad-onnx_b200/csrc/tc_ptx.cuh
@@ -39,6 +39,23 @@
 __device__ __forceinline__ void fence_proxy_async() { asm volatile("fence.proxy.async.shared::cta;" ::: "memory"); }
 __device__ __forceinline__ void tc_fence_before() { asm volatile("tcgen05.fence::before_thread_sync;" ::: "memory"); }
 __device__ __forceinline__ void tc_fence_after() { asm volatile("tcgen05.fence::after_thread_sync;" ::: "memory"); }
+
+__device__ __forceinline__ uint32_t cluster_ctarank() {
+  uint32_t r;
+  asm volatile("mov.u32 %0, %%cluster_ctarank;" : "=r"(r));
+  return r;
+}
+__device__ __forceinline__ uint32_t mapa_shared(uint32_t addr, uint32_t rank) {
+  uint32_t r;
+  asm volatile("mapa.shared::cluster.u32 %0, %1, %2;" : "=r"(r) : "r"(addr), "r"(rank));
+  return r;
+}
+__device__ __forceinline__ void mbar_arrive_cluster(uint32_t cluster_bar) {
+  asm volatile("mbarrier.arrive.shared::cluster.b64 _, [%0];" ::"r"(cluster_bar) : "memory");
+}
+__device__ __forceinline__ void cluster_sync() {
+  asm volatile("barrier.cluster.arrive.release;\nbarrier.cluster.wait.acquire;" ::: "memory");
+}
 
 __device__ __forceinline__ void bulk_g2s(uint32_t dst, const void* src, uint32_t bytes, uint32_t bar) {
   asm volatile("cp.async.bulk.shared::cluster.global.mbarrier::complete_tx::bytes [%0], [%1], %2, [%3];" ::"r"(dst),
@@ -67,16 +84,16 @@
   d |= (uint64_t)1 << 46;
   return d;
 }
-__device__ __forceinline__ uint32_t umma_idesc_bf16(int n) {
-  return (1u << 4) | (1u << 7) | (1u << 10) | ((uint32_t)(n >> 3) << 17) | ((uint32_t)(kTcBM >> 4) << 24);
-}
-__device__ __forceinline__ uint32_t umma_idesc_f16(int n) {
-  return (1u << 4) | ((uint32_t)(n >> 3) << 17) | ((uint32_t)(kTcBM >> 4) << 24);
-}
-__device__ __forceinline__ void umma_bf16(uint32_t tmem_d, uint64_t adesc, uint64_t bdesc, uint32_t idesc,
+__device__ __forceinline__ uint32_t umma_idesc_bf16(int n, int m = kTcBM) {
+  return (1u << 4) | (1u << 7) | (1u << 10) | ((uint32_t)(n >> 3) << 17) | ((uint32_t)(m >> 4) << 24);
+}
+__device__ __forceinline__ uint32_t umma_idesc_f16(int n, int m = kTcBM) {
+  return (1u << 4) | ((uint32_t)(n >> 3) << 17) | ((uint32_t)(m >> 4) << 24);
+}
+__device__ __forceinline__ void umma_pair(uint32_t tmem_d, uint64_t adesc, uint64_t bdesc, uint32_t idesc,
                                           uint32_t accumulate) {
   asm volatile(
-      "{\n.reg .pred p;\nsetp.ne.b32 p, %4, 0;\ntcgen05.mma.cta_group::1.kind::f16 [%0], %1, %2, %3, p;\n}\n" ::"r"(tmem_d),
+      "{\n.reg .pred p;\nsetp.ne.b32 p, %4, 0;\ntcgen05.mma.cta_group::2.kind::f16 [%0], %1, %2, %3, p;\n}\n" ::"r"(tmem_d),
       "l"(adesc), "l"(bdesc), "r"(idesc), "r"(accumulate)
       : "memory");
 }
@@ -105,19 +122,19 @@
       "l"(adesc), "l"(bdesc), "r"(idesc), "r"(accumulate_first), "r"(n_steps)
       : "memory");
 }
-__device__ __forceinline__ void umma_x2(uint32_t tmem_d, uint64_t adesc0, uint64_t adesc1, uint64_t bdesc, uint32_t idesc,
+__device__ __forceinline__ void umma_pair_x2(uint32_t tmem_d, uint64_t adesc0, uint64_t adesc1, uint64_t bdesc, uint32_t idesc,
                                         uint32_t accumulate_first) {
   asm volatile(
       "{\n.reg .pred p, pt;\n"
       "setp.ne.b32 p, %5, 0;\n"
       "setp.eq.b32 pt, 0, 0;\n"
-      "tcgen05.mma.cta_group::1.kind::f16 [%0], %1, %3, %4, p;\n"
-      "tcgen05.mma.cta_group::1.kind::f16 [%0], %2, %3, %4, pt;\n"
+      "tcgen05.mma.cta_group::2.kind::f16 [%0], %1, %3, %4, p;\n"
+      "tcgen05.mma.cta_group::2.kind::f16 [%0], %2, %3, %4, pt;\n"
       "}\n" ::"r"(tmem_d),
       "l"(adesc0), "l"(adesc1), "l"(bdesc), "r"(idesc), "r"(accumulate_first)
       : "memory");
 }
-__device__ __forceinline__ void umma_split_x3(uint32_t tmem_d, uint64_t a, uint32_t a_step, uint32_t a_lo, uint64_t b0,
+__device__ __forceinline__ void umma_pair_split_x3(uint32_t tmem_d, uint64_t a, uint32_t a_step, uint32_t a_lo, uint64_t b0,
                                               uint64_t b1, uint64_t b2, uint32_t idesc, uint32_t accumulate_first,
                                               int n_pairs, uint32_t lo_on) {
   asm volatile(
@@ -138,12 +155,12 @@
       "add.u64 a1h, a1, lo;\n"
       "add.u64 a2, a1, st;\n"
       "add.u64 a2h, a2, lo;\n"
-      "tcgen05.mma.cta_group::1.kind::f16 [%0], %1, %4, %6, p0;\n"
-      "@l0 tcgen05.mma.cta_group::1.kind::f16 [%0], a0h, %4, %6, pt;\n"
-      "@q1 tcgen05.mma.cta_group::1.kind::f16 [%0], a1, %5, %6, pt;\n"
-      "@l1 tcgen05.mma.cta_group::1.kind::f16 [%0], a1h, %5, %6, pt;\n"
-      "@q2 tcgen05.mma.cta_group::1.kind::f16 [%0], a2, %10, %6, pt;\n"
-      "@l2 tcgen05.mma.cta_group::1.kind::f16 [%0], a2h, %10, %6, pt;\n"
+      "tcgen05.mma.cta_group::2.kind::f16 [%0], %1, %4, %6, p0;\n"
+      "@l0 tcgen05.mma.cta_group::2.kind::f16 [%0], a0h, %4, %6, pt;\n"
+      "@q1 tcgen05.mma.cta_group::2.kind::f16 [%0], a1, %5, %6, pt;\n"
+      "@l1 tcgen05.mma.cta_group::2.kind::f16 [%0], a1h, %5, %6, pt;\n"
+      "@q2 tcgen05.mma.cta_group::2.kind::f16 [%0], a2, %10, %6, pt;\n"
+      "@l2 tcgen05.mma.cta_group::2.kind::f16 [%0], a2h, %10, %6, pt;\n"
       "}\n" ::"r"(tmem_d),
       "l"(a), "r"(a_step), "r"(a_lo), "l"(b0), "l"(b1), "r"(idesc), "r"(accumulate_first), "r"(n_pairs), "r"(lo_on),
       "l"(b2)
@@ -151,6 +168,11 @@
 }
 __device__ __forceinline__ void umma_commit(uint32_t bar) {
   asm volatile("tcgen05.commit.cta_group::1.mbarrier::arrive::one.shared::cluster.b64 [%0];" ::"r"(bar) : "memory");
+}
+__device__ __forceinline__ void umma_pair_commit_mc(uint32_t bar) {
+  asm volatile("tcgen05.commit.cta_group::2.mbarrier::arrive::one.shared::cluster.multicast::cluster.b64 [%0], %1;" ::"r"(bar),
+               "h"((uint16_t)3)
+               : "memory");
 }
 __device__ __forceinline__ void tmem_ld16(uint32_t taddr, float* v) {
   uint32_t r[16];
```

Result: no change. 370.9, median of 6 (-0.6%).
